# GATB/dsk

Measured on AMD Instinct MI355X. Metric: distinct k-mers counted/sec (whole node), k=31, higher is better.
Workload: dtype u64

## Files before the change

### dsk_amd/csrc/kernels.h

```cpp
#pragma once
#include "layouts.h"

#ifndef SC_NT
#define SC_NT 1024
#endif
template <int W> struct Tile {
    static constexpr int KPT = 16 / W;
    static constexpr int KEYS = SC_NT * KPT;
    static constexpr int WORDS = KEYS / 32;
};
#define MAX_BINS 2048


template <bool ALIGNED>
__global__ __launch_bounds__(256) void k_encode(const uint8_t* __restrict__ s, u64 n,
                                                u64* __restrict__ packed, u32* __restrict__ inval, u64 nwords) {
    const u64 stride = (u64)gridDim.x * blockDim.x;
    for (u64 w = (u64)blockIdx.x * blockDim.x + threadIdx.x; w < nwords; w += stride) {
        const u64 base = w * 32;
        u32 x[8];
        if (ALIGNED && base + 32 <= n) {
            const uint4 a = *reinterpret_cast<const uint4*>(s + base);
            const uint4 b = *reinterpret_cast<const uint4*>(s + base + 16);
            x[0] = a.x; x[1] = a.y; x[2] = a.z; x[3] = a.w; x[4] = b.x; x[5] = b.y; x[6] = b.z; x[7] = b.w;
// ... 884 lines not shown
                    }
                    s += c[j];
                }
                const u32 inc = wave_incl_scan(s);
                if (lane == 63) wsum[wave] = inc;
                lds_barrier();
                if (wave == 0) {
                    const u32 x = lane < SC_NT / 64 ? wsum[lane] : 0u;
                    const u32 y = wave_incl_scan(x);
                    if (lane < SC_NT / 64) wsum[lane] = y - x;
                    if (lane == SC_NT / 64 - 1) rec[P].z = y;
                }
                lds_barrier();
                u32 run = wsum[wave] + inc - s;
#pragma unroll
                for (int j = 0; j < 4; ++j) {
                    const int b = base + j;
                    if (j < ipt && b < (int)P) { rec[b] = make_uint3(pe[j], er[j], run); run += c[j]; }
                }
            }
            lds_barrier();
            {
                u32 so[KPT];
#pragma unroll
                for (int j = 0; j < KPT; ++j) so[j] = rec[rk[j] >> 16].z;
#pragma unroll
                for (int j = 0; j < KPT; ++j) stage[so[j] + (rk[j] & 0xFFFFu)] = h[j];
            }
            if (tnext < lend) vm = load(tnext, h);
            lds_barrier();
            {
                const u32 nb = wsum[17 + par] < (u32)AL_BIG ? wsum[17 + par] : (u32)AL_BIG;
                for (u32 x = 0; x < nb; ++x) {
                    const uint3 rbig = rec[big[par * AL_BIG + x]];
                    const u32 e = rbig.y & 0x7FFFu, r = rbig.y >> 16, o = rbig.z;
                    const u32 pl = OPT ? rbig.x & ~CHAIN_BIT : rbig.x;
                    Key* ob = (OPT && (rbig.x >> 31)) ? extb : out;
                    for (u32 idx = G + tid; idx < e; idx += SC_NT) ob[pl + idx] = stage[o + idx - r];
                }
            }
            for (u32 b0 = 0; b0 < P; b0 += 2 * NGRP) {
                uint3 rb[2]; u32 rnew[2]; bool act[2];
#pragma unroll
                for (int u = 0; u < 2; ++u) {
                    const u32 b = b0 + u * NGRP + gi;
                    act[u] = b < P;
                    rb[u] = rec[act[u] ? b : 0]; rnew[u] = rn[act[u] ? b : 0];
                }
#pragma unroll
                for (int u = 0; u < 2; ++u) {
                    if (!act[u]) continue;
                    const u32 b = b0 + u * NGRP + gi;
                    const u32 e = rb[u].y & 0x7FFFu, r = rb[u].y >> 16, o = rb[u].z;
                    const u32 mine = (e > AL_BIG_KEYS && !(rb[u].y & 0x8000u)) ? (u32)G : e;
                    const u32 pold = OPT ? rb[u].x & ~CHAIN_BIT : rb[u].x;
                    Key* ob = (OPT && (rb[u].x >> 31)) ? extb : out;
                    Key* cb = carry + (size_t)b * CARRY;
                    for (u32 a = (pold & ~(u32)(G - 1)) + gl; a < pold + mine; a += G) {
                        if (a >= pold) {
                            const u32 idx = a - pold;
                            const Key kv = idx < r ? cb[idx] : stage[o + idx - r];
                            ob[a] = kv;
                        }
                    }
                    const u32 c = rnew[u] + e - r;
                    if (e) { if (gl < rnew[u]) cb[gl] = stage[o + c - rnew[u] + gl]; }
                    else if (gl < c) cb[r + gl] = stage[o + gl];
                }
            }
            par ^= 1u;
        };
        if (lbeg < lend) vm = load(lbeg, h);
        lds_barrier();
        for (u64 t0 = lbeg; t0 < lend; t0 += (u64)TKEYS) process(t0 + TKEYS);
        lds_barrier();
        for (u32 b = gi; b < P; b += NGRP) {
            const u32 r = rn[b];
            if (!OPT) { if (gl < r) out[pos[b] + gl] = carry[(size_t)b * CARRY + gl]; }
            else {
                const u32 p = pos[b], pl = p & ~CHAIN_BIT;
                const bool ext = (p >> 31) != 0u;
                const u32 rs = ext ? pl / os.cap * os.cap : b * os.cap;
                Key* ob = ext ? extb : out;
                if (r) ob[pl + gl] = gl < r ? carry[(size_t)b * CARRY + gl] : empty_key<W>();
                if (gl == 0) os.subcnt[ext ? os.F + pl / os.cap : d.flat_base + b] = pl - rs + r;
            }
        }
        if (OPT && ovf) *os.ovf = 1u;
        if (OPT && os.dbg && tid == 0) os.dbg[3 * g + 1] = wall_clock64();
        if (OPT && os.work) {
            lds_barrier();
            if (tid == 0) wsum[19] = atomicAdd(os.work, 1u);
            lds_barrier();
            g = wsum[19];
        } else g += gridDim.x;
    }
}

struct SegInfo { u32 start, nch, chunk_base, pad; };

__global__ __launch_bounds__(1024) void k_plan(const u32* __restrict__ src, u32 sstride, u32 S, u32 CH, u32 P,
                                               SegInfo* __restrict__ seg, ChunkDesc* __restrict__ descs,
                                               u32* __restrict__ d_nchunks, u32* __restrict__ d_mlen, u32 opt) {
    __shared__ u32 ws[16]; __shared__ u32 carry_s;
    const int lane = threadIdx.x & 63, wave = threadIdx.x >> 6;
    if (threadIdx.x == 0) carry_s = 0;
    __syncthreads();
    for (u32 s0 = 0; s0 < S; s0 += 1024) {
        const u32 s = s0 + threadIdx.x;
        u32 start = 0, size = 0, nch = 0;
        if (s < S) { start = src[(u64)s * sstride]; size = src[(u64)(s + 1) * sstride] - start; nch = (size + CH - 1) / CH; }
        u32 y = nch;
#pragma unroll
        for (int d = 1; d < 64; d <<= 1) { const u32 t = __shfl_up(y, d); if (lane >= d) y += t; }
        if (lane == 63) ws[wave] = y;
        __syncthreads();
        if (wave == 0) {
            const u32 wx = lane < 16 ? ws[lane] : 0u; u32 wy = wx;
#pragma unroll
            for (int d = 1; d < 16; d <<= 1) { const u32 t = __shfl_up(wy, d); if (lane >= d) wy += t; }
            if (lane < 16) ws[lane] = wy - wx;
        }
        __syncthreads();
        const u32 cb = carry_s + ws[wave] + y - nch;
        if (s < S) {
            SegInfo si; si.start = start; si.nch = nch; si.chunk_base = cb; si.pad = 0;
            seg[s] = si;
            for (u32 c = 0; c < nch; ++c) {
                ChunkDesc d;
                d.begin = (u64)start + (u64)c * CH;
                const u64 e = d.begin + CH, lim = (u64)start + size;
                d.end = e < lim ? e : lim;
                d.flat_base = opt ? s * P : cb * P + c;
                d.stride = nch;
                descs[cb + c] = d;
            }
        }
        __syncthreads();
        if (threadIdx.x == 1023) carry_s = cb + nch;
        __syncthreads();
    }
    if (threadIdx.x == 0) { *d_nchunks = carry_s; *d_mlen = carry_s * P; }
}

__global__ void k_final_offsets(const u32* __restrict__ scanned, const SegInfo* __restrict__ seg,
                                u32 P, u32 stride1, const u32* __restrict__ d_mlen,
                                u32* __restrict__ fstart, u32 F) {
    const u32 q = blockIdx.x * blockDim.x + threadIdx.x;
    if (q > F) return;
    if (seg == nullptr) { fstart[q] = scanned[(u64)q * stride1]; return; }
    if (q == F) { fstart[q] = scanned[*d_mlen]; return; }
    const u32 s = q / P, b = q % P;
    const SegInfo si = seg[s];
    fstart[q] = si.nch ? scanned[(u64)si.chunk_base * P + (u64)b * si.nch] : si.start;
}

#ifndef CNT_NT
#define CNT_NT 1024
#endif
#define CNT_SLOTS 4096
#define CNT_MAXLOAD 3584
#define CNT_LH 512
#ifndef CNT_KPT
#define CNT_KPT 3
#endif

struct CountParams {
    u32 F;
    u32 amin, amax, histo_max;
    u32 maxload;
    u32 cap;
    const u32* subcnt;
};
template <bool REG>
__device__ __forceinline__ void sub_range(const CountParams& cp, const u32* __restrict__ fstart, u32 q, u64* begin, u32* n) {
    if (REG) { *begin = (u64)q * cp.cap; *n = cp.subcnt[q]; }
    else { const u32 b = fstart[q]; *begin = b; *n = fstart[q + 1] - b; }
}

__device__ __forceinline__ void table_insert1(u64* tk, u32* tc, unsigned short* lst, u32* ndist, u32* ovf, u64 h, u32 inc = 1u) {
    u32 slot = (u32)h & (CNT_SLOTS - 1);
    int probe = 0;
    for (; probe < CNT_SLOTS; ++probe) {
        u64 old = tk[slot];
        if (old == DSK_EMPTY) {
            old = atomicCAS(&tk[slot], DSK_EMPTY, h);
            if (old == DSK_EMPTY) { lst[atomicAdd(ndist, 1u)] = (unsigned short)slot; old = h; }
        }
        if (old == h) { atomicAdd(&tc[slot], inc); return; }
        slot = (slot + 1) & (CNT_SLOTS - 1);
    }
    *ovf = 1;
}

template <bool REG>
__global__ __launch_bounds__(CNT_NT) void k_count1(u64* keys, u64* solid_keys, const u32* __restrict__ fstart,
                                                    u32* __restrict__ abund, u32* __restrict__ nsolid,
                                                    u64* __restrict__ ghist, u64* __restrict__ gstats,
                                                    u32* __restrict__ overflow, CountParams cp, const u32* __restrict__ subcnt) {
    __shared__ u64 tk[CNT_SLOTS];
    __shared__ u32 tc[CNT_SLOTS];
    __shared__ unsigned short lst[CNT_SLOTS];
    __shared__ u32 lh[CNT_LH];
    __shared__ u32 s_ctr[2][4];
    const int tid = threadIdx.x, lane = tid & 63;
    for (int s = tid; s < CNT_SLOTS; s += CNT_NT) { tk[s] = DSK_EMPTY; tc[s] = 0; }
    for (int b = tid; b < CNT_LH; b += CNT_NT) lh[b] = 0;
    if (tid < 8) s_ctr[tid >> 2][tid & 3] = 0;
    u32 ones = 0;
    u64 ndist_acc = 0;
    auto range_lo = [&](u32 qq) { const u32 c = qq < cp.F ? qq : cp.F - 1; return REG ? subcnt[c] : fstart[c]; };
    auto range_hi = [&](u32 qq) { const u32 c = qq < cp.F ? qq : cp.F - 1; return REG ? 0u : fstart[c + 1]; };
    auto begin_of = [&](u32 qq, u32 lo) { return REG ? (u64)qq * cp.cap : (u64)lo; };
    auto count_of = [&](u32 qq, u32 lo, u32 hi) { return qq < cp.F ? (REG ? ((int)lo < 0 ? 0u : lo) : hi - lo) : 0u; };
    struct Sub { u32 q; u64 begin; u32 n; };
    auto load_keys = [&](const Sub& sb, u64 (&pk)[CNT_KPT]) {
        const u32 last = sb.n ? sb.n - 1 : 0u;
#pragma unroll
        for (int j = 0; j < CNT_KPT; ++j) { const u32 i = tid + j * CNT_NT; pk[j] = keys[sb.begin + (i < sb.n ? i : last)]; }
    };
    auto sub_of = [&](u32 qq, u32 lo, u32 hi) { Sub sb; sb.q = qq; sb.begin = qq < cp.F ? begin_of(qq, lo) : 0ull; sb.n = count_of(qq, lo, hi); return sb; };
    const u32 G = gridDim.x;
    u64 pa[CNT_KPT], pb[CNT_KPT];
    Sub sa = sub_of(blockIdx.x, range_lo(blockIdx.x), range_hi(blockIdx.x));
    Sub sb = sub_of(blockIdx.x + G, range_lo(blockIdx.x + G), range_hi(blockIdx.x + G));
    u32 rq = blockIdx.x + 2 * G, rlo = range_lo(rq), rhi = range_hi(rq);
    load_keys(sa, pa);
    load_keys(sb, pb);
    lds_barrier();
    int par = 0;
    auto one = [&](Sub& cur, u64 (&pk)[CNT_KPT]) {
        u32* ctr = s_ctr[par];
        const u32 q = cur.q, n = cur.n; const u64 begin = cur.begin;
#pragma unroll
        for (int j = 0; j < CNT_KPT; ++j)
            if ((u32)(tid + j * CNT_NT) < n) table_insert1(tk, tc, lst, &ctr[0], &ctr[2], pk[j]);
        for (u32 i = CNT_KPT * CNT_NT + tid; i < n; i += CNT_NT)
            table_insert1(tk, tc, lst, &ctr[0], &ctr[2], keys[begin + i]);
        cur = sub_of(rq, rlo, rhi);
        load_keys(cur, pk);
        rq += G; rlo = range_lo(rq); rhi = range_hi(rq);
        lds_barrier();
        const u32 nd = ctr[0];
        const bool bad = ctr[2] || nd > cp.maxload;
        if (bad) {
            for (int s = tid; s < CNT_SLOTS; s += CNT_NT) { tk[s] = DSK_EMPTY; tc[s] = 0; }
            if (tid == 0) *overflow = 1;
        } else {
            for (u32 i0 = 0; i0 < nd; i0 += CNT_NT) {
                const u32 i = i0 + tid;
                const bool act = i < nd;
                u64 key = 0; u32 c = 0;
                if (act) {
                    const u32 slot = lst[i];
                    key = tk[slot]; c = tc[slot];
                    tk[slot] = DSK_EMPTY; tc[slot] = 0;
                }
                const u64 m1 = __ballot(act && c == 1);
                if (lane == 0) ones += __popcll(m1);
                if (act && c > 1) {
                    const u32 bin = c < cp.histo_max ? c : cp.histo_max;
                    if (bin < CNT_LH) atomicAdd(&lh[bin], 1u);
                    else atomicAdd(&ghist[bin], 1ull);
                }
                const bool solid = act && c >= cp.amin && c <= cp.amax;
                const u64 ms = __ballot(solid);
                if (ms) {
                    u32 base = 0;
                    if (lane == 0) base = atomicAdd(&ctr[1], (u32)__popcll(ms));
                    base = __shfl(base, 0);
                    if (solid) {
                        const u32 pos = base + __popcll(ms & ((1ull << lane) - 1));
                        solid_keys[begin + pos] = key;
                        abund[begin + pos] = c;
                    }
                }
            }
        }
        lds_barrier();
        if (tid == 0) {
            nsolid[q] = bad ? 0u : ctr[1];
            ndist_acc += bad ? 0u : nd;
            ctr[0] = 0; ctr[1] = 0; ctr[2] = 0;
        }
        par ^= 1;
    };
    while (sa.q < cp.F) {
        one(sa, pa);
        if (sb.q >= cp.F) break;
        one(sb, pb);
    }
    lds_barrier();
    if (lane == 0 && ones) atomicAdd(&lh[1], ones);
    lds_barrier();
    for (int b = tid; b < CNT_LH; b += CNT_NT) {
        const u32 v = lh[b];
        if (v) atomicAdd(&ghist[b < (int)cp.histo_max ? b : (int)cp.histo_max], (u64)v);
    }
    if (tid == 0 && ndist_acc) atomicAdd(&gstats[0], ndist_acc);
}

#define CNT_V3_KEYS 5
#define CNT_NONE 0xFFFFFFFFu
__device__ __forceinline__ u32 table_insert3(u64* tk, u32* tc, u32* ovf, u64 h) {
    u32 slot = (u32)h & (CNT_SLOTS - 1), res = CNT_NONE;
    bool pend = true;
    for (int probe = 0; probe < CNT_SLOTS; ++probe) {
        u64 old = 0ull;
        if (pend) old = tk[slot];
        const bool e = pend && old == DSK_EMPTY;
        if (e) { old = atomicCAS(&tk[slot], DSK_EMPTY, h); if (old == DSK_EMPTY) { res = slot; old = h; } }
        const bool m = pend && old == h;
        if (m) atomicAdd(&tc[slot], 1u);
        pend = pend && !m;
        slot = (slot + 1) & (CNT_SLOTS - 1);
        if (!__ballot(pend)) return res;
    }
    *ovf = 1;
    return res;
}

template <int NT, int KPT, int NKEYS>
__global__ __launch_bounds__(NT) void k_count1v3(u64* keys, u64* solid_keys, u32* __restrict__ abund, u32* __restrict__ nsolid,
                                                      u64* __restrict__ ghist, u64* __restrict__ gstats,
                                                      u32* __restrict__ overflow, CountParams cp, const u32* __restrict__ subcnt) {
    __shared__ u64 tk[CNT_SLOTS];
    __shared__ u32 tc[CNT_SLOTS];
    __shared__ u32 lh[CNT_LH];
    __shared__ u32 s_ctr[2][4];
    const int tid = threadIdx.x, lane = tid & 63;
    for (int s = tid; s < CNT_SLOTS; s += NT) { tk[s] = DSK_EMPTY; tc[s] = 0; }
    for (int b = tid; b < CNT_LH; b += NT) lh[b] = 0;
    if (tid < 8) s_ctr[tid >> 2][tid & 3] = 0;
    u32 ones = 0;
    u64 ndist_acc = 0;
    auto range_lo = [&](u32 qq) { const u32 c = qq < cp.F ? qq : cp.F - 1; return subcnt[c]; };
    auto count_of = [&](u32 qq, u32 lo) { return qq < cp.F ? ((int)lo < 0 ? 0u : lo) : 0u; };
    struct Sub { u32 q; u64 begin; u32 n; };
    auto load_keys = [&](const Sub& sb, u64 (&pk)[KPT]) {
        const u32 last = sb.n ? sb.n - 1 : 0u;
#pragma unroll
        for (int j = 0; j < KPT; ++j) { const u32 i = tid + j * NT; pk[j] = keys[sb.begin + (i < sb.n ? i : last)]; }
    };
    auto sub_of = [&](u32 qq, u32 lo) { Sub sb; sb.q = qq; sb.begin = qq < cp.F ? (u64)qq * cp.cap : 0ull; sb.n = count_of(qq, lo); return sb; };
    const u32 G = gridDim.x;
    u64 pa[KPT], pb[KPT];
    Sub sa = sub_of(blockIdx.x, range_lo(blockIdx.x));
    Sub sb = sub_of(blockIdx.x + G, range_lo(blockIdx.x + G));
    u32 rq = blockIdx.x + 2 * G, rlo = range_lo(rq);
    load_keys(sa, pa);
    load_keys(sb, pb);
    lds_barrier();
    int par = 0;
    auto one = [&](Sub& cur, u64 (&pk)[KPT]) {
        u32* ctr = s_ctr[par];
        const u32 q = cur.q, n = cur.n; const u64 begin = cur.begin;
        u32 cl[NKEYS];
#pragma unroll
        for (int j = 0; j < NKEYS; ++j) cl[j] = CNT_NONE;
#pragma unroll
        for (int j = 0; j < KPT; ++j)
            if ((u32)(tid + j * NT) < n) cl[j] = table_insert3(tk, tc, &ctr[2], pk[j]);
#pragma unroll
        for (int j = KPT; j < NKEYS; ++j)
            if ((u32)(tid + j * NT) < n) cl[j] = table_insert3(tk, tc, &ctr[2], keys[begin + tid + j * NT]);
        {
            u32 mine = 0;
#pragma unroll
            for (int j = 0; j < NKEYS; ++j) mine += (u32)__popcll(__ballot(cl[j] != CNT_NONE));
            if (lane == 0 && mine) atomicAdd(&ctr[0], mine);
        }
        cur = sub_of(rq, rlo);
        load_keys(cur, pk);
        rq += G; rlo = range_lo(rq);
        lds_barrier();
        const u32 nd = ctr[0];
        const bool bad = ctr[2] || nd > cp.maxload;
        if (bad) {
            for (int s = tid; s < CNT_SLOTS; s += NT) { tk[s] = DSK_EMPTY; tc[s] = 0; }
            if (tid == 0) *overflow = 1;
        } else {
#pragma unroll
            for (int j = 0; j < NKEYS; ++j) {
                const bool act = cl[j] != CNT_NONE;
                if (!__ballot(act)) continue;
                u64 key = 0; u32 c = 0;
                if (act) {
                    const u32 slot = cl[j];
                    key = tk[slot]; c = tc[slot];
                    tk[slot] = DSK_EMPTY; tc[slot] = 0;
                }
                const u64 m1 = __ballot(act && c == 1);
                if (lane == 0) ones += __popcll(m1);
                if (act && c > 1) {
                    const u32 bin = c < cp.histo_max ? c : cp.histo_max;
                    if (bin < CNT_LH) atomicAdd(&lh[bin], 1u);
                    else atomicAdd(&ghist[bin], 1ull);
                }
                const bool solid = act && c >= cp.amin && c <= cp.amax;
                const u64 ms = __ballot(solid);
                if (ms) {
                    u32 base = 0;
                    if (lane == 0) base = atomicAdd(&ctr[1], (u32)__popcll(ms));
                    base = __shfl(base, 0);
                    if (solid) {
                        const u32 pos = base + __popcll(ms & ((1ull << lane) - 1));
                        solid_keys[begin + pos] = key;
                        abund[begin + pos] = c;
                    }
                }
            }
        }
        lds_barrier();
        if (tid == 0) {
            nsolid[q] = bad ? 0u : ctr[1];
            ndist_acc += bad ? 0u : nd;
            ctr[0] = 0; ctr[1] = 0; ctr[2] = 0;
        }
        par ^= 1;
    };
    while (sa.q < cp.F) {
        one(sa, pa);
        if (sb.q >= cp.F) break;
        one(sb, pb);
    }
    lds_barrier();
    if (lane == 0 && ones) atomicAdd(&lh[1], ones);
    lds_barrier();
    for (int b = tid; b < CNT_LH; b += NT) {
        const u32 v = lh[b];
        if (v) atomicAdd(&ghist[b < (int)cp.histo_max ? b : (int)cp.histo_max], (u64)v);
    }
    if (tid == 0 && ndist_acc) atomicAdd(&gstats[0], ndist_acc);
}

__global__ __launch_bounds__(CNT_NT) void k_count_chained(u64* keys, u64* solid_keys, u32* __restrict__ abund, u32* __restrict__ nsolid,
                                                          u64* __restrict__ ghist, u64* __restrict__ gstats, u32* __restrict__ overflow,
                                                          CountParams cp, const u32* __restrict__ subcnt, const u32* __restrict__ chain_next,
                                                          const u32* __restrict__ chain_list, const u32* __restrict__ d_nchained, u32 list_cap) {
    __shared__ u64 tk[CNT_SLOTS];
    __shared__ u32 tc[CNT_SLOTS];
    __shared__ unsigned short lst[CNT_SLOTS];
    __shared__ u32 lh[CNT_LH];
    __shared__ u32 ctr[4];
    const int tid = threadIdx.x, lane = tid & 63;
    const u32 nchained = *d_nchained < list_cap ? *d_nchained : list_cap;
    if (blockIdx.x >= nchained) return;
    for (int s = tid; s < CNT_SLOTS; s += CNT_NT) { tk[s] = DSK_EMPTY; tc[s] = 0; }
    for (int b = tid; b < CNT_LH; b += CNT_NT) lh[b] = 0;
    if (tid < 4) ctr[tid] = 0;
    u32 ones = 0;
    u64 ndist_acc = 0;
    __syncthreads();
    for (u32 li = blockIdx.x; li < nchained; li += gridDim.x) {
        const u32 q = chain_list[li];
        const u64 begin = (u64)q * cp.cap;
        u32 rg = q;
        while (true) {
            const u32 f = subcnt[rg], nn = f & ~CHAIN_BIT;
            const u64 rb = (u64)rg * cp.cap;
            for (u32 i0 = 0; i0 < nn; i0 += CNT_NT) {
                const bool act = i0 + tid < nn;
                const u64 kv = keys[rb + (act ? i0 + tid : 0u)];
                const u64 first = ((u64)__builtin_amdgcn_readfirstlane((u32)(kv >> 32)) << 32) | __builtin_amdgcn_readfirstlane((u32)kv);
                const bool same = act && kv == first;
                const u64 m = __ballot(same);
                if (same && lane == __ffsll((unsigned long long)m) - 1) table_insert1(tk, tc, lst, &ctr[0], &ctr[2], first, (u32)__popcll(m));
                if (act && !same) table_insert1(tk, tc, lst, &ctr[0], &ctr[2], kv);
            }
            if (!(f >> 31)) break;
            rg = chain_next[rg];
        }
        __syncthreads();
        const u32 nd = ctr[0];
        const bool bad = ctr[2] || nd > cp.maxload;
        if (bad) {
            for (int s = tid; s < CNT_SLOTS; s += CNT_NT) { tk[s] = DSK_EMPTY; tc[s] = 0; }
            if (tid == 0) *overflow = 1;
        } else {
            for (u32 i0 = 0; i0 < nd; i0 += CNT_NT) {
                const u32 i = i0 + tid;
                const bool act = i < nd;
                u64 key = 0; u32 c = 0;
                if (act) {
                    const u32 slot = lst[i];
                    key = tk[slot]; c = tc[slot];
                    tk[slot] = DSK_EMPTY; tc[slot] = 0;
                }
                const u64 m1 = __ballot(act && c == 1);
                if (lane == 0) ones += __popcll(m1);
                if (act && c > 1) {
                    const u32 bin = c < cp.histo_max ? c : cp.histo_max;
                    if (bin < CNT_LH) atomicAdd(&lh[bin], 1u);
                    else atomicAdd(&ghist[bin], 1ull);
                }
                const bool solid = act && c >= cp.amin && c <= cp.amax;
                const u64 ms = __ballot(solid);
                if (ms) {
                    u32 base = 0;
                    if (lane == 0) base = atomicAdd(&ctr[1], (u32)__popcll(ms));
                    base = __shfl(base, 0);
                    if (solid) {
                        const u32 pos = base + __popcll(ms & ((1ull << lane) - 1));
                        solid_keys[begin + pos] = key;
                        abund[begin + pos] = c;
                    }
                }
            }
        }
        __syncthreads();
        if (tid == 0) {
            nsolid[q] = bad ? 0u : ctr[1];
            ndist_acc += bad ? 0u : nd;
            ctr[0] = 0; ctr[1] = 0; ctr[2] = 0;
        }
        __syncthreads();
    }
    if (lane == 0 && ones) atomicAdd(&lh[1], ones);
    __syncthreads();
    for (int b = tid; b < CNT_LH; b += CNT_NT) {
        const u32 v = lh[b];
        if (v) atomicAdd(&ghist[b < (int)cp.histo_max ? b : (int)cp.histo_max], (u64)v);
    }
    if (tid == 0 && ndist_acc) atomicAdd(&gstats[0], ndist_acc);
}

#define C2_SLOTS 4096
#define C2_MAXLOAD 3584
template <int W> struct CStage { static constexpr int N = 4096 / W; static constexpr int KPT = N / CNT_NT; };

template <int W>
__device__ __forceinline__ void table_insert2(const KN<W>* sk, const KN<W>* __restrict__ gkeys, u32* slots, u32* tc,
                                              unsigned short* lst, u32* ndist, u32* ovf, const KN<W>& key, u32 idx) {
    constexpr u32 C2_STAGE = CStage<W>::N;
    u32 slot = (u32)key.w[W - 1] & (C2_SLOTS - 1);
    for (int probe = 0; probe < C2_SLOTS; ++probe) {
        u32 v = slots[slot];
        if (v == 0) {
            v = atomicCAS(&slots[slot], 0u, idx + 1);
            if (v == 0) { lst[atomicAdd(ndist, 1u)] = (unsigned short)slot; atomicAdd(&tc[slot], 1u); return; }
        }
        const u32 r = v - 1;
        bool same = true;
        if (W == 2) {
            KN<W> rep;
            if (r < C2_STAGE) rep = sk[r]; else rep = gkeys[r];
            same = key_eq(rep, key);
        } else if (r < C2_STAGE) {
#pragma unroll
            for (int x = 0; x < W; ++x) same = same && (sk[r].w[x] == key.w[x]);
        } else {
#pragma unroll
            for (int x = 0; x < W; ++x) same = same && (gkeys[r].w[x] == key.w[x]);
        }
        if (same) { atomicAdd(&tc[slot], 1u); return; }
        slot = (slot + 1) & (C2_SLOTS - 1);
    }
    *ovf = 1;
}

template <int W, bool REG>
__global__ __launch_bounds__(CNT_NT) void k_count_mw(KN<W>* keys, KN<W>* solid_keys, const u32* __restrict__ fstart,
                                                     u32* __restrict__ abund, u32* __restrict__ nsolid,
                                                     u64* __restrict__ ghist, u64* __restrict__ gstats,
                                                     u32* __restrict__ overflow, CountParams cp) {
    typedef KN<W> K2;
    constexpr int C2_STAGE = CStage<W>::N, C2_KPT = CStage<W>::KPT;
    __shared__ K2 sk[C2_STAGE];
    __shared__ u32 slots[C2_SLOTS];
    __shared__ u32 tc[C2_SLOTS];
    __shared__ unsigned short lst[C2_SLOTS];
    __shared__ u32 lh[CNT_LH];
    __shared__ u32 ctr[4];
    const int tid = threadIdx.x, lane = tid & 63;
    for (int s = tid; s < C2_SLOTS; s += CNT_NT) { slots[s] = 0; tc[s] = 0; }
    for (int b = tid; b < CNT_LH; b += CNT_NT) lh[b] = 0;
    if (tid < 4) ctr[tid] = 0;
    u32 ones = 0; u64 ndist_acc = 0;
    u32 q = blockIdx.x, begin = 0, end = 0;
    K2 pk[C2_KPT];
    if (q < cp.F) {
        if (REG) { const u32 c = cp.subcnt[q]; begin = q * cp.cap; end = begin + ((int)c < 0 ? 0u : c); } else { begin = fstart[q]; end = fstart[q + 1]; }
#pragma unroll
        for (int j = 0; j < C2_KPT; ++j) { const u32 i = begin + tid + j * CNT_NT; if (i < end) pk[j] = keys[i]; }
    }
    lds_barrier();
    while (q < cp.F) {
        const u32 n = end - begin;
        const K2* gk = keys + begin;
#pragma unroll
        for (int j = 0; j < C2_KPT; ++j) { const u32 i = tid + j * CNT_NT; if (i < n) sk[i] = pk[j]; }
        lds_barrier();
#pragma unroll
        for (int j = 0; j < C2_KPT; ++j) {
            const u32 i = tid + j * CNT_NT;
            if (i < n) table_insert2(sk, gk, slots, tc, lst, &ctr[0], &ctr[2], pk[j], i);
        }
        for (u32 i = C2_STAGE + tid; i < n; i += CNT_NT) {
            const K2 kx = gk[i];
            table_insert2(sk, gk, slots, tc, lst, &ctr[0], &ctr[2], kx, i);
        }
        const u32 qn = q + gridDim.x;
        u32 nbeg = 0, nend = 0;
        if (qn < cp.F) {
            if (REG) { const u32 c = cp.subcnt[qn]; nbeg = qn * cp.cap; nend = nbeg + ((int)c < 0 ? 0u : c); } else { nbeg = fstart[qn]; nend = fstart[qn + 1]; }
#pragma unroll
            for (int j = 0; j < C2_KPT; ++j) { const u32 i = nbeg + tid + j * CNT_NT; if (i < nend) pk[j] = keys[i]; }
        }
        lds_barrier();
        const u32 nd = ctr[0];
        const bool bad = ctr[2] || nd > cp.maxload;
        if (bad) {
            for (int s = tid; s < C2_SLOTS; s += CNT_NT) { slots[s] = 0; tc[s] = 0; }
            if (tid == 0) *overflow = 1;
        } else {
            for (u32 i0 = 0; i0 < nd; i0 += CNT_NT) {
                const u32 i = i0 + tid;
                const bool act = i < nd;
                u64 kw[W]; u32 c = 0;
#pragma unroll
                for (int x = 0; x < W; ++x) kw[x] = 0;
                if (act) {
                    const u32 slot = lst[i];
                    const u32 r = slots[slot] - 1;
                    if (W == 2) {
                        K2 key; if (r < C2_STAGE) key = sk[r]; else key = gk[r];
#pragma unroll
                        for (int x = 0; x < W; ++x) kw[x] = key.w[x];
                    } else if (r < C2_STAGE) {
#pragma unroll
                        for (int x = 0; x < W; ++x) kw[x] = sk[r].w[x];
                    } else {
#pragma unroll
                        for (int x = 0; x < W; ++x) kw[x] = gk[r].w[x];
                    }
                    c = tc[slot];
                    slots[slot] = 0; tc[slot] = 0;
                }
                const u64 m1 = __ballot(act && c == 1);
                if (lane == 0) ones += __popcll(m1);
                if (act && c > 1) {
                    const u32 bin = c < cp.histo_max ? c : cp.histo_max;
                    if (bin < CNT_LH) atomicAdd(&lh[bin], 1u);
                    else atomicAdd(&ghist[bin], 1ull);
                }
                const bool solid = act && c >= cp.amin && c <= cp.amax;
                const u64 ms = __ballot(solid);
                if (ms) {
                    u32 base = 0;
                    if (lane == 0) base = atomicAdd(&ctr[1], (u32)__popcll(ms));
                    base = __shfl(base, 0);
                    if (solid) {
                        const u32 pos = base + __popcll(ms & ((1ull << lane) - 1));
#pragma unroll
                        for (int x = 0; x < W; ++x) solid_keys[begin + pos].w[x] = kw[x];
                        abund[begin + pos] = c;
                    }
                }
            }
        }
        lds_barrier();
        if (tid == 0) {
            nsolid[q] = bad ? 0u : ctr[1];
            ndist_acc += bad ? 0u : nd;
            ctr[0] = 0; ctr[1] = 0; ctr[2] = 0;
        }
        q = qn; begin = nbeg; end = nend;
    }
    lds_barrier();
    if (lane == 0 && ones) atomicAdd(&lh[1], ones);
    lds_barrier();
    for (int b = tid; b < CNT_LH; b += CNT_NT) {
        const u32 v = lh[b];
        if (v) atomicAdd(&ghist[b < (int)cp.histo_max ? b : (int)cp.histo_max], (u64)v);
    }
    if (tid == 0 && ndist_acc) atomicAdd(&gstats[0], ndist_acc);
}

#define C2V_SLOTS 3072
#define C2V_MAXLOAD 2688
#define C2V_NKEYS 4
#define C2V_KPT 2
#define CNT_OVF_VERIFY 2u
#define CNT_OVF_SENTINEL 4u
__device__ __forceinline__ u32 table_insert3w(u64* tk, u64* tl, u32* tc, u32* ovf, u64 top, u64 low) {
    u32 slot = (u32)(((u64)(u32)top * C2V_SLOTS) >> 32), res = CNT_NONE;
    bool pend = true;
    for (int probe = 0; probe < C2V_SLOTS; ++probe) {
        u64 old = 0ull;
        if (pend) old = tk[slot];
        const bool e = pend && old == DSK_EMPTY;
        u32 mine = 0u;
        if (e) { old = atomicCAS(&tk[slot], DSK_EMPTY, top); if (old == DSK_EMPTY) { mine = 0x80000000u; old = top; tl[slot] = low; } }
// ... 533 lines not shown
```

Baseline: 26.81 billion.

## Resize count-kernel hash table, add per-thread key queue insertion and occupancy hint

Makes the LDS hash table size a template parameter, defaulting to 6144 slots with a multiply-high home-slot mapping for non-power-of-two sizes. It adds an optional packed 16-bit count mode, off by default. It also adds a queue-style insert, on by default, where each lane moves to its next key as soon as the current one is placed, so lanes do not sit idle waiting on the slowest key per round. A min-blocks launch bound is added to raise occupancy. The risks are more register pressure from shifting key arrays and a changed table load factor, which affects probe lengths and overflow fallbacks.

Result: faster. 27.42 billion (median of 6 runs) (+2.3%).

```diff
diff --git a/dsk_amd/csrc/kernels.h b/dsk_amd/csrc/kernels.h
--- a/dsk_amd/csrc/kernels.h
+++ b/dsk_amd/csrc/kernels.h
@@ -1210,34 +1210,93 @@
 
 #define CNT_V3_KEYS 5
 #define CNT_NONE 0xFFFFFFFFu
+#ifndef CNT_V3_SLOTS
+#define CNT_V3_SLOTS 6144
+#endif
+#ifndef CNT_V3_PACK
+#define CNT_V3_PACK false
+#endif
+#ifndef CNT_V3_QUEUE
+#define CNT_V3_QUEUE true
+#endif
+template <int SLOTS> __device__ __forceinline__ u32 cnt_home(u64 h) {
+    if constexpr ((SLOTS & (SLOTS - 1)) == 0) return (u32)h & (SLOTS - 1);
+    else return __umulhi(__builtin_rotateleft32((u32)h, 20), (u32)SLOTS);
+}
+template <int SLOTS> __device__ __forceinline__ u32 cnt_next(u32 slot) {
+    if constexpr ((SLOTS & (SLOTS - 1)) == 0) return (slot + 1) & (SLOTS - 1);
+    else return slot + 1 == SLOTS ? 0u : slot + 1;
+}
+template <bool PACK> __device__ __forceinline__ void cnt_add(u32* tc, u32 slot) {
+    if constexpr (PACK) atomicAdd(&tc[slot >> 1], 1u << ((slot & 1) * 16));
+    else atomicAdd(&tc[slot], 1u);
+}
+template <int SLOTS = CNT_SLOTS, bool PACK = false>
 __device__ __forceinline__ u32 table_insert3(u64* tk, u32* tc, u32* ovf, u64 h) {
-    u32 slot = (u32)h & (CNT_SLOTS - 1), res = CNT_NONE;
+    u32 slot = cnt_home<SLOTS>(h), res = CNT_NONE;
     bool pend = true;
-    for (int probe = 0; probe < CNT_SLOTS; ++probe) {
+    for (int probe = 0; probe < SLOTS; ++probe) {
         u64 old = 0ull;
         if (pend) old = tk[slot];
         const bool e = pend && old == DSK_EMPTY;
         if (e) { old = atomicCAS(&tk[slot], DSK_EMPTY, h); if (old == DSK_EMPTY) { res = slot; old = h; } }
         const bool m = pend && old == h;
-        if (m) atomicAdd(&tc[slot], 1u);
+        if (m) cnt_add<PACK>(tc, slot);
         pend = pend && !m;
-        slot = (slot + 1) & (CNT_SLOTS - 1);
+        slot = cnt_next<SLOTS>(slot);
         if (!__ballot(pend)) return res;
     }
     *ovf = 1;
     return res;
 }
-
-template <int NT, int KPT, int NKEYS>
-__global__ __launch_bounds__(NT) void k_count1v3(u64* keys, u64* solid_keys, u32* __restrict__ abund, u32* __restrict__ nsolid,
+template <int KPT, int SLOTS, bool PACK, int NCL>
+__device__ __forceinline__ void table_insert_queue(u64* tk, u32* tc, u32* ovf, u64 (&pk)[KPT], u32 nk, u32 (&cl)[NCL]) {
+    u32 left = nk, slot = cnt_home<SLOTS>(pk[0]);
+    for (int round = 0; round < KPT * SLOTS; ++round) {
+        const bool pend = left != 0;
+        const u64 h = pk[0];
+        u64 old = 0ull;
+        if (pend) old = tk[slot];
+        const bool e = pend && old == DSK_EMPTY;
+        if (e) {
+            old = atomicCAS(&tk[slot], DSK_EMPTY, h);
+            if (old == DSK_EMPTY) {
+#pragma unroll
+                for (int j = KPT - 1; j > 0; --j) cl[j] = cl[j - 1];
+                cl[0] = slot; old = h;
+            }
+        }
+        const bool m = pend && old == h;
+        const u32 nxt = cnt_next<SLOTS>(slot);
+        if (m) {
+            cnt_add<PACK>(tc, slot);
+            --left;
+#pragma unroll
+            for (int j = 0; j + 1 < KPT; ++j) pk[j] = pk[j + 1];
+        }
+        slot = m ? cnt_home<SLOTS>(pk[0]) : nxt;
+        if (!__ballot(left != 0)) return;
+    }
+    *ovf = 1;
+}
+
+template <int NT, int KPT, int NKEYS, int SLOTS = CNT_V3_SLOTS, bool PACK = CNT_V3_PACK, bool QUEUE = CNT_V3_QUEUE>
+__global__ __launch_bounds__(NT, NT / 128) void k_count1v3(u64* keys, u64* solid_keys, u32* __restrict__ abund, u32* __restrict__ nsolid,
                                                       u64* __restrict__ ghist, u64* __restrict__ gstats,
                                                       u32* __restrict__ overflow, CountParams cp, const u32* __restrict__ subcnt) {
-    __shared__ u64 tk[CNT_SLOTS];
-    __shared__ u32 tc[CNT_SLOTS];
+    static_assert(NKEYS * NT < 65536 || !PACK, "a packed count holds a region's keys");
+    static_assert(SLOTS % 2 == 0 && KPT <= NKEYS, "table shape");
+    constexpr int NCW = PACK ? SLOTS / 2 : SLOTS;
+    __shared__ u64 tk[SLOTS];
+    __shared__ u32 tc[NCW];
     __shared__ u32 lh[CNT_LH];
     __shared__ u32 s_ctr[2][4];
     const int tid = threadIdx.x, lane = tid & 63;
-    for (int s = tid; s < CNT_SLOTS; s += NT) { tk[s] = DSK_EMPTY; tc[s] = 0; }
+    auto clear_table = [&]() {
+        for (int s = tid; s < SLOTS; s += NT) tk[s] = DSK_EMPTY;
+        for (int s = tid; s < NCW; s += NT) tc[s] = 0;
+    };
+    clear_table();
     for (int b = tid; b < CNT_LH; b += NT) lh[b] = 0;
     if (tid < 8) s_ctr[tid >> 2][tid & 3] = 0;
     u32 ones = 0;
@@ -1266,12 +1325,19 @@
         u32 cl[NKEYS];
 #pragma unroll
         for (int j = 0; j < NKEYS; ++j) cl[j] = CNT_NONE;
-#pragma unroll
-        for (int j = 0; j < KPT; ++j)
-            if ((u32)(tid + j * NT) < n) cl[j] = table_insert3(tk, tc, &ctr[2], pk[j]);
+        if constexpr (QUEUE) {
+            u32 nk = 0;
+#pragma unroll
+            for (int j = 0; j < KPT; ++j) nk += (u32)(tid + j * NT) < n ? 1u : 0u;
+            if (n) table_insert_queue<KPT, SLOTS, PACK>(tk, tc, &ctr[2], pk, nk, cl);
+        } else {
+#pragma unroll
+            for (int j = 0; j < KPT; ++j)
+                if ((u32)(tid + j * NT) < n) cl[j] = table_insert3<SLOTS, PACK>(tk, tc, &ctr[2], pk[j]);
+        }
 #pragma unroll
         for (int j = KPT; j < NKEYS; ++j)
-            if ((u32)(tid + j * NT) < n) cl[j] = table_insert3(tk, tc, &ctr[2], keys[begin + tid + j * NT]);
+            if ((u32)(tid + j * NT) < n) cl[j] = table_insert3<SLOTS, PACK>(tk, tc, &ctr[2], keys[begin + tid + j * NT]);
         {
             u32 mine = 0;
 #pragma unroll
@@ -1285,7 +1351,7 @@
         const u32 nd = ctr[0];
         const bool bad = ctr[2] || nd > cp.maxload;
         if (bad) {
-            for (int s = tid; s < CNT_SLOTS; s += NT) { tk[s] = DSK_EMPTY; tc[s] = 0; }
+            clear_table();
             if (tid == 0) *overflow = 1;
         } else {
 #pragma unroll
@@ -1295,8 +1361,11 @@
                 u64 key = 0; u32 c = 0;
                 if (act) {
                     const u32 slot = cl[j];
-                    key = tk[slot]; c = tc[slot];
-                    tk[slot] = DSK_EMPTY; tc[slot] = 0;
+                    key = tk[slot]; tk[slot] = DSK_EMPTY;
+                    if constexpr (PACK) {
+                        const u32 sh = (slot & 1) * 16;
+                        c = (atomicAnd(&tc[slot >> 1], 0xFFFF0000u >> sh) >> sh) & 0xFFFFu;
+                    } else { c = tc[slot]; tc[slot] = 0; }
                 }
                 const u64 m1 = __ballot(act && c == 1);
                 if (lane == 0) ones += __popcll(m1);
```
